# kris927b/TextBlaster

Hardware: AMD Instinct MI355X
Metric: documents/sec through full C4+Gopher+langID pipeline at 1/2/4/8 MI355X (higher is better)
Workload: dtype bf16

## Files before the change

csrc/common/docproc.h:

```cpp
#pragma once
#include <type_traits>

#include "devplan.h"
#include "hash.h"
#include "langid.h"
#include "par.h"
#include "uax29.h"
#include "ucd.h"

namespace tb {

enum : int {
  PH_START = 0, PH_DECODE, PH_DICT, PH_PREFIX_HASH, PH_WORDS, PH_LINES, PH_GQ, PH_GR_LINES, PH_GR_WORDS,
  PH_GR_TOP, PH_GR_DUP, PH_FW, PH_LID, PH_GR_DUP_WALK, PH_GR_DUP_CANON, PH_GR_TOP_CANON,
  PH_C4_LOREM = 16, PH_C4_DECODE, PH_C4_LINES, PH_C4_CITE, PH_C4_WORDS, PH_C4_CODES, PH_C4_JOIN, PH_C4_SENT,
  PH_GR_NL = 24, PH_GR_LINE_DUP, PH_GR_WH, PH_GR_WCANON, PH_GQ_WORDS, PH_GQ_BYTES, PH_RUST_LINES,
  kPhaseSlots = 32
};

enum : uint32_t {
  DOC_OK = 0,
  DOC_NEEDS_CPU = 1,
  DOC_OVERFLOW = 2,
};
// ... 729 lines not shown
  bool collided = false;
  x.par.for_n(n, [&](uint32_t i) {
    uint32_t c = (uint32_t)(tab[canon[i]] & 0xFFFFFFFFull) - 1u;
    if (c != i && !eq(i, c)) { collided = true; c = i; }
    canon[i] = c;
    res(i, c);
  });
  if (collided) x.set_flag(DOC_NEEDS_CPU);
  x.par.sync();
  x.reset(mark);
}

template <class P, class KeyF, class EqF, class CT>
TB_HD void canonicalize(DocCtx<P>& x, uint32_t n, KeyF&& key, EqF&& eq, CT* canon) {
  canonicalize_res(x, n, key, eq, canon, NoResolve{});
}

template <class P>
TB_HD bool bytes_eq(const uint8_t* b, uint32_t a0, uint32_t a1, uint32_t b0, uint32_t b1) {
  if (a1 - a0 != b1 - b0) return false;
  const uint32_t n = a1 - a0;
  uint32_t i = 0;
  for (; i + 16 <= n; i += 16) {
    uint32_t diff = 0;
#pragma unroll
    for (uint32_t k = 0; k < 16; ++k) diff |= (uint32_t)(b[a0 + i + k] ^ b[b0 + i + k]);
    if (diff) return false;
  }
  uint32_t diff = 0;
  for (; i < n; ++i) diff |= (uint32_t)(b[a0 + i] ^ b[b0 + i]);
  return diff == 0;
}

template <class P, class SpanF>
TB_HD void dup_spans(DocCtx<P>& x, const uint8_t* b, const PHView& ph, uint32_t n, SpanF&& span,
                     int64_t* out_elems, int64_t* out_bytes) {
  if (n <= 1) {
    *out_elems = 0;
    *out_bytes = 0;
    return;
  }
  const auto mark = x.mark();
  uint32_t* canon = x.template alloc_hot<uint32_t>(n + 1);
  if (x.overflow) return;
  canonicalize(
      x, n,
      [&](uint32_t i) {
        uint32_t s, e;
        span(i, s, e);
        return dev_key(span_hash8(x, ph, s, e), e - s);
      },
      [&](uint32_t i, uint32_t j) {
        uint32_t s0, e0, s1, e1;
        span(i, s0, e0);
        span(j, s1, e1);
        return bytes_eq<P>(b, s0, e0, s1, e1);
      },
      canon);
  *out_elems = x.par.template sum<int64_t>(n, [&](uint32_t i) { return canon[i] != i ? (int64_t)1 : (int64_t)0; });
  *out_bytes = x.par.template sum<int64_t>(n, [&](uint32_t i) {
    if (canon[i] == i) return (int64_t)0;
    uint32_t s, e;
    span(i, s, e);
    return (int64_t)(e - s);
  });
  x.reset(mark);
}

template <class F>
TB_HD void lower_bytes(const UcdView& ucd, const Cps& cv, uint32_t s, uint32_t e, F&& push) {
  uint8_t buf[4];
  const PropArr prop = cv.props();
  for (uint32_t k = s; k < e; ++k) {
    uint32_t c = cv.cp(k);
    uint32_t lc;
    if (c == 0x3A3) {
      bool before = false, after = false;
      for (uint32_t j = k; j > s; --j) {
        uint32_t p = prop[j - 1];
        if (p & P16_CASE_IGN) continue;
        before = (p & P_CASED) != 0;
        break;
      }
// ... 310 lines not shown
  uint32_t* segf = x.template alloc_hot<uint32_t>(kChunk + 1);
  if (x.overflow) return 0;
  const PropArr prop = c.props() + s;
  CpsAcc acc{prop};
  uint32_t cnt = 0;
  bool seen = false;
  for (uint32_t base = 0; base < m && cnt < limit; base += kChunk) {
    const uint32_t len = m - base < kChunk ? m - base : kChunk;
    const uint32_t NS = x.par.template compact<int>(
        len, [&](uint32_t i, int&) { const uint32_t g = base + i; return g == 0 || sb_break(acc, (int)m, (int)g); },
        [&](uint32_t i, uint32_t k, int&) { starts[k] = i; });
    x.par.sync();
    const uint32_t first = NS ? starts[0] : len;
    const bool lead_any = x.par.template sum<uint32_t>(first, [&](uint32_t i) {
      return is_ws(prop[base + i]) ? 0u : 1u;
    }) != 0;
    const uint32_t segs = x.par.template sum<uint32_t>(NS, [&](uint32_t k) {
      const uint32_t a = starts[k], bnd = k + 1 < NS ? starts[k + 1] : len;
      uint32_t f = 0;
      for (uint32_t j = a; j < bnd; ++j) if (!is_ws(prop[base + j])) { f = 1; break; }
      segf[k] = f;
      return f;
    });
    x.par.sync();
    if (!seen && lead_any) ++cnt;
    cnt += segs;
    seen = NS ? segf[NS - 1] != 0 : (seen || lead_any);
    x.par.sync();
  }
  x.reset(mark);
  return cnt;
}

template <class P>
TB_HD void gopher_rep_record(DocCtx<P>& x, const DevStep& ds, const uint8_t* b, const Cps& c,
                             const PHView& ph, const Words& w, int64_t* r, bool release_props = false,
                             GrExport* ex = nullptr, const PreDoc* pre = nullptr,
                             const uint8_t* b_export = nullptr, Lines lines = Lines{}) {
  const uint32_t C = c.n;
  const PropArr prop = c.props();
  const OffArr off = c.offs();
  const int width = ds.width;
  uint32_t tcs, tce;
  trim_span(x, prop, C, tcs, tce);
  if (tcs >= tce) {
    x.par.single([&]() {
      for (int k = 0; k < width; ++k) r[k] = 0;
      r[0] = -1;
    });
    return;
  }
  const auto mark = x.mark();
  const uint32_t span = tce - tcs;
  uint32_t* rs;
  uint32_t* rl;
  uint32_t NR;
  if (pre) {
    const uint32_t a = pre->nl_a, e = pre->nl_e;
    rs = pre->nl_pos + a;
    rl = pre->nl_len + a;
    NR = e - a;
  } else if (lines.n > 0) {
    const uint32_t* ls = lines.ls;
    const uint32_t NL = lines.n;
    rs = P::kWaves == 1 ? x.template alloc_hot<uint32_t>(NL + 1) : x.template alloc<uint32_t>(NL + 1);
    rl = P::kWaves == 1 ? x.template alloc_hot<uint32_t>(NL + 1) : x.template alloc<uint32_t>(NL + 1);
    if (x.overflow) return;
// ... 47 lines not shown
  const uint32_t NPR = x.par.template compact<int>(
      NR, [&](uint32_t k, int&) { return rl[k] >= 2; }, [&](uint32_t k, uint32_t q, int&) { prs[q] = k; });
  x.par.sync();
  if (!split_lines)
    dup_spans(x, b, ph, NPR + 1,
              [&](uint32_t q, uint32_t& s0, uint32_t& e0) {
                gr_para_span(rs, rl, prs, off, tcs, tce, NPR, q, s0, e0);
              },
              &para_dup, &para_dup_b);
  if (ex) {
    x.par.single([&]() {
      ex->rs = rs; ex->rl = rl; ex->prs = prs; ex->off = off; ex->ph = ph;
      ex->NR = NR; ex->NPR = NPR; ex->tcs = tcs; ex->tce = tce;
      ex->lines_valid = split_lines ? 1u : 0u;
    });
  }
  x.stamp(PH_GR_LINES);
  x.par.single([&]() {
    r[0] = span;
    r[1] = NPR + 1;
    r[2] = para_dup;
    r[3] = para_dup_b;
    r[4] = NR + 1;
    r[5] = line_dup;
    r[6] = line_dup_b;
  });
  const uint32_t W = w.n;
  const bool ngrams = ds.n_top + ds.n_dup > 0;
  if constexpr (P::kWaves == 1) {
    if (ngrams && W >= kWave16) {
      x.set_flag(DOC_NEEDS_CPU);
      return;
    }
    if (ngrams && ex) {
      const uint64_t base = (x.used + 255) & ~255ull;
      x.par.single([&]() {
        for (int t = 0; t < ds.n_top + ds.n_dup; ++t) r[rec_gr_fixed() + t] = 0;
        ex->bs = w.bs; ex->be = w.be;
        ex->b = b_export ? b_export : b;
        ex->free_base = x.scr + base;
        ex->free_cap = x.cap > base ? x.cap - base : 0;
        ex->W = W;
        ex->valid = x.overflow ? 0u : 1u;
      });
      x.par.sync();
      x.stamp(PH_GR_WORDS);
      x.reset(mark);
      return;
    }
  }
  uint32_t* wid = nullptr;
  uint32_t* WL = nullptr;
  uint64_t* K = nullptr;
  uint64_t* PB = nullptr;
  if (ngrams && pre && pre->wready) {
    wid = pre->wid;
    WL = pre->wl;
    K = pre->wk;
    PB = pre->wpb;
  } else if (ngrams) {
    const uint64_t tab_bytes = 6ull * W + 64;
    wid = ex ? x.template alloc<uint32_t>(W + 1) : x.template alloc_hot_keep<uint32_t>(W + 1, tab_bytes);
    WL = ex ? x.template alloc<uint32_t>(W + 1) : x.template alloc_hot_keep<uint32_t>(W + 1, tab_bytes);
    K = ex ? x.template alloc<uint64_t>(W + 1) : x.template alloc_hot_keep<uint64_t>(W + 1, tab_bytes);
    PB = ex ? x.template alloc<uint64_t>(W + 1) : x.template alloc_hot_keep<uint64_t>(W + 1, tab_bytes);
    const auto mw = x.mark();
    uint64_t* wh = x.template alloc_hot_hi<uint64_t>(W + 1);
    if (x.overflow) return;
    x.par.for_n(W, [&](uint32_t k) { wh[k] = span_hash8(x, ph, w.bs[k], w.be[k]); });
    x.par.sync();
    x.stamp(PH_GR_WH);
    canonicalize(
        x, W, [&](uint32_t k) { return dev_key(wh[k], w.be[k] - w.bs[k]); },
        [&](uint32_t i, uint32_t j) { return bytes_eq<P>(b, w.bs[i], w.be[i], w.bs[j], w.be[j]); }, wid);
    x.stamp(PH_GR_WCANON);
    const uint32_t totl = x.par.template scan<uint32_t>(
        W, 0u, [](uint32_t a, uint32_t c2) { return a + c2; },
        [&](uint32_t k) { return w.be[k] - w.bs[k]; }, [&](uint32_t k, uint32_t e) { WL[k] = e; });
    x.par.single([&]() { WL[W] = totl; });
    x.par.sync();
    x.par.for_n(W + 1, [&](uint32_t k) { PB[k] = x.powb(WL[k]); });
    const uint64_t ktot = x.par.template scan<uint64_t>(
        W, 0ull, [](uint64_t a, uint64_t c2) { return a + c2; },
        [&](uint32_t j) { return wh[j] * x.ipowb(WL[j + 1]); }, [&](uint32_t k, uint64_t e) { K[k] = e; });
    x.par.single([&]() { K[W] = ktot; });
    x.par.sync();
    x.reset(mw);
    if (x.overflow) return;
  }
  x.stamp(PH_GR_WORDS);
  if (release_props) x.release_hi();
  if (ngrams) {
    const DupGrams dg{wid, WL, K, PB, w.bs, w.be, b};
    if (ds.n_top > 0 && ex) {
      x.par.single([&]() { for (int t = 0; t < ds.n_top; ++t) r[rec_gr_fixed() + t] = 0; });
    } else if (ds.n_top > 0) {
      int max_top = 0;
      for (int t = 0; t < ds.n_top; ++t) max_top = ds.top_n[t] > max_top ? ds.top_n[t] : max_top;
      const auto m2 = x.mark();
      uint32_t* ga = x.template alloc_hot_keep<uint32_t>(W + 1, 6ull * W + 64);
      uint32_t* gb = x.template alloc_hot_keep<uint32_t>(W + 1, 6ull * W + 64);
      if (x.overflow) return;
      x.par.single([&]() { for (int t = 0; t < ds.n_top; ++t) r[rec_gr_fixed() + t] = 0; });
      const uint32_t* gprev = wid;
      for (uint32_t n = 1; n <= (uint32_t)max_top && W >= n; ++n) {
        const uint32_t G = W - n + 1;
        const uint32_t* gc = wid;
        uint32_t* cnt = (n == 1 || !(n & 1)) ? ga : gb;
        if (n > 1) {
          uint32_t* gcur = (n & 1) ? ga : gb;
          canonicalize(
              x, G, [&](uint32_t p) { return mix64(((uint64_t)gprev[p] << 32) ^ (uint64_t)wid[p + n - 1] ^ ((uint64_t)n << 60)); },
              [&](uint32_t p, uint32_t q) { return gprev[p] == gprev[q] && wid[p + n - 1] == wid[q + n - 1]; }, gcur);
          gc = gcur;
          gprev = gcur;
          x.stamp(PH_GR_TOP_CANON);
        }
        bool wanted = false;
        for (int t = 0; t < ds.n_top; ++t) wanted |= ds.top_n[t] == (int32_t)n;
        if (!wanted) continue;
        x.par.for_n(G, [&](uint32_t p) { cnt[p] = 0; });
        x.par.sync();
        x.par.for_n(G, [&](uint32_t p) { P::add32(&cnt[gc[p]], 1u); });
        x.par.sync();
        const uint32_t maxc = x.par.template max<uint32_t>(G, 0u, [&](uint32_t p) { return cnt[p]; });
        int64_t v = 0;
        if (maxc > 1) {
          const uint32_t maxlen = x.par.template max<uint32_t>(G, 0u, [&](uint32_t p) {
            return cnt[p] == maxc ? (WL[p + n] - WL[p] + n - 1) : 0u;
          });
          v = (int64_t)maxlen * (int64_t)maxc;
        }
        x.par.single([&]() {
          for (int t = 0; t < ds.n_top; ++t) if (ds.top_n[t] == (int32_t)n) r[rec_gr_fixed() + t] = v;
        });
        x.par.sync();
      }
      x.reset(m2);
    }
    x.stamp(PH_GR_TOP);
    if (ex) {
      const uint64_t base = (x.used + 255) & ~255ull;
      x.par.single([&]() {
        for (int t = 0; t < ds.n_dup; ++t) r[rec_gr_fixed() + ds.n_top + t] = 0;
        ex->wid = wid; ex->WL = WL; ex->K = K; ex->PB = PB; ex->bs = w.bs; ex->be = w.be;
        ex->b = b_export ? b_export : b;
        ex->free_base = x.scr + base;
        ex->free_cap = x.cap > base ? x.cap - base : 0;
        ex->W = W;
        ex->valid = x.overflow ? 0u : 1u;
      });
      x.par.sync();
    } else if (ds.n_dup > 0) {
      const uint32_t SW = (W + 31) / 32 + 1;
      const int nd = ds.n_dup;
      auto gsize = [&](int t) -> uint32_t {
        const uint32_t n = (uint32_t)ds.dup_n[t];
        return (n == 0 || W < n) ? 0u : W - n + 1;
      };
      uint32_t gtot = 0;
      for (int t = 0; t < nd; ++t) gtot += gsize(t);
      const auto m3 = x.mark();
      uint32_t* bits = x.template alloc_hot<uint32_t>(2 * (uint64_t)SW * (uint64_t)nd);
      using GcT = std::conditional_t<P::kWaves == 1, uint16_t, uint32_t>;
      GcT* gcall = x.template alloc_hot_keep<GcT>((uint64_t)gtot + 1, 6ull * W + 64);
      if (x.overflow) return;
      x.par.for_n(2 * SW * (uint32_t)nd, [&](uint32_t i) { bits[i] = 0; });
      x.par.sync();
      uint32_t gb = 0;
      for (int t = 0; t < nd; ++t) {
        const uint32_t n = (uint32_t)ds.dup_n[t];
        const uint32_t G = gsize(t);
        if (G == 0) continue;
        GcT* gc = gcall + gb;
        uint32_t* R = bits + (uint32_t)t * 2 * SW + SW;
        gb += G;
        auto mark_rep = [&](uint32_t p, uint32_t g) {
          if (g != p) {
            P::or32(&R[p >> 5], 1u << (p & 31));
            P::or32(&R[g >> 5], 1u << (g & 31));
          }
        };
        if constexpr (P::kWaves != 1) {
          canonicalize_res(
              x, G, [&](uint32_t p) { return dg.key(p, n); }, [&](uint32_t p, uint32_t q) { return dg.eq(p, q, n); },
              gc, mark_rep);
          x.stamp(PH_GR_DUP_CANON);
        } else {
          canonicalize(
              x, G, [&](uint32_t p) { return dg.key(p, n); }, [&](uint32_t p, uint32_t q) { return dg.eq(p, q, n); },
              gc);
          x.stamp(PH_GR_DUP_CANON);
          x.par.for_n(G, [&](uint32_t p) { mark_rep(p, gc[p]); });
          x.par.sync();
        }
      }
      auto walk = [&](uint32_t t, bool wave) -> int64_t {
        const uint32_t G = gsize((int)t);
        if (G == 0) return 0;
        uint32_t base = 0;
        for (uint32_t u = 0; u < t; ++u) base += gsize((int)u);
        uint32_t* sn = bits + t * 2 * SW;
        const uint32_t n = (uint32_t)ds.dup_n[t];
        return wave ? dup_walk_wave(x.par, G, n, gcall + base, sn + SW, sn, WL)
                    : dup_walk(G, n, gcall + base, sn + SW, sn, WL);
      };
      if constexpr (P::kWaves > 1) {
        for (uint32_t t = x.par.wave_index(); t < (uint32_t)nd; t += P::kWaves) {
          const int64_t rep = walk(t, true);
          if (x.par.lane == 0) r[rec_gr_fixed() + ds.n_top + t] = rep;
        }
      } else {
        x.par.for_n((uint32_t)nd, [&](uint32_t t) { r[rec_gr_fixed() + ds.n_top + t] = walk(t, false); });
      }
      x.par.sync();
      x.stamp(PH_GR_DUP_WALK);
      x.reset(m3);
      x.stamp(PH_GR_DUP);
    }
  }
  x.reset(mark);
}

template <class P, class KeyF>
TB_HD uint32_t repeat_candidates(DocCtx<P>& x, uint32_t n, KeyF&& key, uint32_t* bm, uint32_t bw, uint32_t* list) {
  const uint32_t mask = bw * 32u - 1u;
  uint32_t* once = bm;
  uint32_t* twice = bm + bw;
  x.par.for_n(2 * bw, [&](uint32_t i) { bm[i] = 0; });
  x.par.sync();
  x.par.for_n(n, [&](uint32_t i) {
    const uint32_t h = (uint32_t)(key(i) >> 20) & mask;
    const uint32_t bit = 1u << (h & 31u);
    if (P::fetch_or32(&once[h >> 5], bit) & bit) P::or32(&twice[h >> 5], bit);
  });
  x.par.sync();
  const uint32_t nc = x.par.template compact<int>(
      n,
      [&](uint32_t i, int&) {
        const uint32_t h = (uint32_t)(key(i) >> 20) & mask;
        return ((twice[h >> 5] >> (h & 31u)) & 1u) != 0;
      },
      [&](uint32_t i, uint32_t k, int&) { list[k] = i; });
  x.par.sync();
  return nc;
}

TB_HD uint32_t cand_bitmap_words(uint32_t n) {
  uint32_t w = 32;
  while (w * 4u < n) w <<= 1;
  return w;
// ... 1032 lines not shown
    x.par.single([&]() { *wout = wk; });
  }
  x.stamp(PH_C4_CODES);
  uint32_t* joff = x.template alloc_hot<uint32_t>(NLn + 1);
  if (x.overflow) { x.set_flag(DOC_NEEDS_CPU | DOC_OVERFLOW); return; }
  uint32_t Jtot = x.par.template scan<uint32_t>(
      NLn, 0u, [](uint32_t a, uint32_t b2) { return a + b2; },
      [&](uint32_t k) { return code[k] == 0 ? plen[k] + 1 : 0u; }, [&](uint32_t k, uint32_t e) { joff[k] = e; });
  if (Jtot > 0) Jtot -= 1;
  uint8_t* Jb = x.template alloc_global<uint8_t>(Jtot + 1);
  if (x.overflow) { x.set_flag(DOC_NEEDS_CPU | DOC_OVERFLOW); return; }
  x.par.sync();
  x.par.for_n(C, [&](uint32_t j) {
    const uint32_t nb = kept_bytes(j);
    if (!nb || code[lid[j]] != 0) return;
    const uint32_t k = lid[j];
    uint8_t* d = Jb + joff[k] + (Pw[j] - Pw[la[k]]);
    for (uint32_t q = 0; q < nb; ++q) d[q] = b[off[j] + q];
  });
  x.par.for_n(NLn, [&](uint32_t k) {
    if (code[k] == 0 && joff[k] + plen[k] < Jtot) Jb[joff[k] + plen[k]] = '\n';
  });
  x.par.sync();
  x.stamp(PH_C4_JOIN);
  c4_finish(x, c4, n, Jb, Jtot, s_long, s_punct, s_few, r, src);
}


#ifndef TB_HOT_PROPS
#define TB_HOT_PROPS 1
#endif
constexpr bool kHotProps = TB_HOT_PROPS != 0;

template <class P, bool kWithLid = true, bool kPre = false>
TB_HD void analyze_stage(DocCtx<P>& x, const DevStage& st, const DevPlan& plan,
                         const LidTables& lid, const uint8_t* b, uint32_t n, StageOut& out) {
  bool need_words = false, need_lines = false, need_ph = false, need_lid = false;
  for (int s = 0; s < st.n_steps; ++s) {
    const int k = st.steps[s].kind;
    if (k == DK_GOPHER_QUALITY) need_words = need_lines = true;
    if (k == DK_GOPHER_REP) need_words = need_ph = true;
    if (k == DK_FINEWEB) need_words = need_lines = need_ph = true;
    if (k == DK_LANGID) need_lid = true;
  }
  x.stamp(PH_START);
  if (out.line_stats) x.par.single([&]() { out.line_stats[0] = kLineStatsNone; });
  uint32_t ndict = 0;
  Cps c;
  if constexpr (kPre) {
    c.n = out.pre->C;
    c.off = out.pre->off;
    c.prop = out.pre->prop;
    c.b = b;
    c.nb = n;
    ndict = out.pre->dict;
  } else {
    c = decode(x, b, n, kHotProps, &ndict);
  }
  if (x.overflow) { x.set_flag(DOC_NEEDS_CPU | DOC_OVERFLOW); return; }
  x.stamp(PH_DECODE);
  const uint32_t C = c.n;
  const uint32_t* dict_marks = nullptr;
  uint32_t wfix = kNoWords;
  if (ndict && need_words) {
    bool fw_only = true;
    for (int s = 0; s < st.n_steps; ++s)
      fw_only &= st.steps[s].kind != DK_GOPHER_QUALITY && st.steps[s].kind != DK_GOPHER_REP;
    if (!kPre) dict_marks = out.dict.marks(out.doc);
    if (!kPre && !dict_marks && fw_only) wfix = out.dict.nwords(out.doc);
    if (!dict_marks && wfix == kNoWords) {
      if constexpr (kWithLid) {
        for (int s = 0; s < st.n_steps; ++s) {
          const DevStep& ds = st.steps[s];
          if (ds.kind == DK_LANGID && lid.E)
            langid_record(x, b, n, lid, out.rec + (int64_t)ds.rec_prefix * out.ndocs + (int64_t)out.doc * ds.width);
        }
      }
      x.set_flag(DOC_NEEDS_CPU);
      return;
    }
  }
  x.stamp(PH_DICT);
  PHView ph;
  if (need_ph) ph = prefix_hash8(x, b, n);
  x.stamp(PH_PREFIX_HASH);
  Words w;
  if (need_words) {
    w = words(x, c, kPre ? out.pre : nullptr, dict_marks);
  }
  x.stamp(PH_WORDS);
  Lines L;
  if (need_lines) L = rust_lines(x, c);
  if (x.overflow) { x.set_flag(DOC_NEEDS_CPU | DOC_OVERFLOW); return; }
  x.stamp(PH_RUST_LINES);
  if (out.line_stats && need_words && need_lines) export_line_stats(x, c, w, L, n, out.line_stats);
  x.stamp(PH_LINES);
  const uint32_t W = w.n;
  const PropArr prop = c.props();
  const OffArr off = c.offs();

  int n_gr = 0;
  for (int s = 0; s < st.n_steps; ++s) n_gr += st.steps[s].kind == DK_GOPHER_REP;
  int gr_seen = 0;
  for (int so = 0; so < 2 * st.n_steps; ++so) {
    const int s = so % st.n_steps;
    const DevStep& ds = st.steps[s];
    if ((so < st.n_steps) == (ds.kind == DK_GOPHER_REP)) continue;
    int64_t* r = out.rec + (int64_t)ds.rec_prefix * out.ndocs + (int64_t)out.doc * ds.width;
    if (ds.kind == DK_GOPHER_QUALITY) {
      const DevStopSet& ss = plan.stops[ds.stop_set];
      const UcdView ucd = x.ucd;
      auto lo32 = [](uint64_t v) { return (int64_t)(v & 0xFFFFFFFFull); };
      auto hi32 = [](uint64_t v) { return (int64_t)(v >> 32); };
      int64_t sum_chars = 0;
      const uint64_t as = x.par.template sum<uint64_t>(W, [&](uint32_t k) {
        const uint32_t a = w.cs[k], e = w.ce[k];
        return ((uint64_t)(e - a) << 32) | ((uint64_t)w.alpha[k] << 16) |
// ... 18 lines not shown
        if (c0 == 0xE2) return (uint64_t)(i + 2 < n && b[i + 1] == 0x80 && b[i + 2] == 0xA6);
        if (c0 != '.' || (i > 0 && b[i - 1] == '.')) return (uint64_t)0;
        uint32_t j = i;
        while (j < n && b[j] == '.') ++j;
        return (uint64_t)((j - i) / 3);
      });
      x.stamp(PH_GQ_BYTES);
      const int64_t nhash = hi32(he), nell = lo32(he);
      const uint64_t be = x.par.template sum<uint64_t>(L.n, [&](uint32_t k) {
        const uint32_t ls = L.ls[k], le = L.le[k];
        uint32_t j = ls;
        while (j < le && is_ws(prop[j])) ++j;
        const uint32_t l0 = j < le ? c.lead(j) : 0u;
        const uint64_t bul = (l0 == '-' || (l0 == 0xE2 && c.cp(j) == 0x2022)) ? 1 : 0;
        j = le;
        while (j > ls && is_ws(prop[j - 1])) --j;
        const uint32_t E = off[j], S = off[ls];
        uint64_t ell = 0;
        if (E - S >= 3) {
          const bool dots = b[E - 3] == '.' && b[E - 2] == '.' && b[E - 1] == '.';
          const bool uell = b[E - 3] == 0xE2 && b[E - 2] == 0x80 && b[E - 1] == 0xA6;
          ell = (dots || uell) ? 1 : 0;
        }
        return (bul << 32) | ell;
      });
      const int64_t bullet = hi32(be), ell_lines = lo32(be);
      x.par.single([&]() {
        r[0] = W; r[1] = sum_chars; r[2] = nhash; r[3] = nell; r[4] = L.n;
        r[5] = bullet; r[6] = ell_lines; r[7] = alpha; r[8] = stop;
      });
      x.stamp(PH_GQ);
    } else if (ds.kind == DK_GOPHER_REP) {
      ++gr_seen;
      gopher_rep_record(x, ds, b, c, ph, w, r, kHotProps && gr_seen == n_gr, n_gr == 1 ? out.gr_export : nullptr,
                        kPre ? out.pre : nullptr, out.b_global, L);
    } else if (ds.kind == DK_FINEWEB) {
      const auto mark = x.mark();
      uint32_t* nb = x.template alloc<uint32_t>(L.n + 1);
      if (x.overflow) { x.set_flag(DOC_NEEDS_CPU | DOC_OVERFLOW); return; }
      const uint32_t NB = x.par.template compact<int>(
          L.n,
          [&](uint32_t k, int&) {
            for (uint32_t j = L.ls[k]; j < L.le[k]; ++j) if (!is_ws(prop[j])) return true;
            return false;
          },
          [&](uint32_t k, uint32_t q, int&) { nb[q] = k; });
      x.par.sync();
      int64_t stop_end = x.par.template sum<int64_t>(NB, [&](uint32_t q) {
        uint32_t k = nb[q];
        uint32_t j = L.le[k];
        while (j > L.ls[k] && is_ws(prop[j - 1])) --j;
        uint32_t last = c.cp(j - 1);
        for (int t = 0; t < ds.n_stop_chars; ++t) if (ds.stop_chars[t] == last) return (int64_t)1;
        return (int64_t)0;
      });
      int64_t shrt = x.par.template sum<int64_t>(NB, [&](uint32_t q) {
        uint32_t k = nb[q];
        return (int64_t)((int64_t)(L.le[k] - L.ls[k]) <= ds.short_line_length);
      });
      int64_t dup_e = 0, dup_b = 0;
      dup_spans(x, b, ph, NB,
                [&](uint32_t q, uint32_t& s0, uint32_t& e0) { s0 = off[L.ls[nb[q]]]; e0 = off[L.le[nb[q]]]; },
                &dup_e, &dup_b);
      int64_t nl = x.par.template sum<int64_t>(C, [&](uint32_t i) { return (int64_t)c.is_lf(i); });
      x.par.single([&]() {
        r[0] = NB; r[1] = stop_end; r[2] = shrt; r[3] = dup_b; r[4] = (int64_t)C - nl; r[5] = nl; r[6] = W;
      });
      x.reset(mark);
// ... 22 lines not shown
```

csrc/hip/stage.hip:

```cpp
#include <algorithm>

#include "kernel_common.h"

namespace {

#define TB_STAGE_KERNEL(NAME, ATTR)                                                                   \
  __global__ __launch_bounds__(64) ATTR void NAME(                                                   \
      const DevPlan* __restrict__ plan, const DevStage* __restrict__ stage, const uint8_t* __restrict__ bytes, \
      const int64_t* __restrict__ off, const int32_t* __restrict__ perm, int32_t ndocs, char* scratch,        \
      const int64_t* __restrict__ scratch_off, const uint64_t* __restrict__ pw, uint32_t pw_n, DevTables tabs, \
      int64_t* rec, uint32_t* flags, uint32_t lds_bytes, uint64_t* prof,                               \
      const uint8_t* __restrict__ dead, uint32_t* line_stats, GrExport* gr_export, DictIn dict) {      \
    const int doc = perm ? perm[blockIdx.x] : (int)blockIdx.x;                                        \
    if (doc >= ndocs || (dead && dead[doc])) return;                                                  \
    DocCtx<WavePar> x = make_ctx(tabs, pw, pw_n, scratch, scratch_off, doc, (int)blockIdx.x, flags, lds_bytes, prof);   \
    const uint32_t n = (uint32_t)(off[doc + 1] - off[doc]);                                           \
    lds_ascii_props(x);                                                                               \
    const uint8_t* b = lds_text(x, bytes + off[doc], n);                                              \
    StageOut out{rec, (uint32_t)ndocs, (uint32_t)doc};                                                \
    if (line_stats) out.line_stats = line_stats + line_stats_base(off[doc], doc);                     \
    if (gr_export) { out.gr_export = gr_export + blockIdx.x; out.b_global = bytes + off[doc]; }       \
    out.dict = dict;                                                                                  \
    analyze_stage<WavePar, false>(x, *stage, *plan, LidTables{}, b, n, out);  \
  }

#ifndef TB_STAGE_WPE
#define TB_STAGE_WPE 8
#endif
TB_STAGE_KERNEL(k_stage_analyze_wave, __attribute__((amdgpu_waves_per_eu(TB_STAGE_WPE, 8))))

#ifndef TB_BLK_WPE
#define TB_BLK_WPE 6
#endif
#if TB_BLK_WPE > 0
#define TB_BLK_ATTR __attribute__((amdgpu_waves_per_eu(TB_BLK_WPE, 8)))
#else
#define TB_BLK_ATTR
#endif

template <int NT, bool kPre = false>
__device__ __forceinline__ void stage_blk_body(
    const DevPlan* __restrict__ plan, const DevStage* __restrict__ stage, const uint8_t* __restrict__ bytes,
    const int64_t* __restrict__ off, const int32_t* __restrict__ perm, int32_t ndocs, char* scratch,
    const int64_t* __restrict__ scratch_off, const uint64_t* __restrict__ pw, uint32_t pw_n, DevTables tabs,
    int64_t* rec, uint32_t* flags, uint32_t lds_bytes, uint64_t* prof, const uint8_t* __restrict__ dead,
    GrExport* gr_export, int32_t n_split, uint32_t split_bytes, uint32_t* line_stats, const PreDoc* pre,
    int32_t n_pre, DictIn dict) {
  const int doc = perm[blockIdx.x];
  if (doc >= ndocs || (dead && dead[doc])) return;
  DocCtx<BlockPar<NT>> x =
      make_ctx<BlockPar<NT>>(tabs, pw, pw_n, scratch, scratch_off, doc, (int)blockIdx.x, flags, lds_bytes, prof);
  x.par.xs = g_block_xs;
  lds_ascii_props(x);
  const uint8_t* b = bytes + off[doc];
  const uint32_t n = (uint32_t)(off[doc + 1] - off[doc]);
  StageOut out{rec, (uint32_t)ndocs, (uint32_t)doc};
  out.dict = dict;
  if (line_stats) out.line_stats = line_stats + line_stats_base(off[doc], doc);
  if constexpr (kPre) {
    if (pre[blockIdx.x].n != n) return;
    out.pre = pre + blockIdx.x;
  }
// ... 7 lines not shown
      const int64_t* __restrict__ off, const int32_t* __restrict__ perm, int32_t ndocs, char* scratch,         \
      const int64_t* __restrict__ scratch_off, const uint64_t* __restrict__ pw, uint32_t pw_n, DevTables tabs,  \
      int64_t* rec, uint32_t* flags, uint32_t lds_bytes, uint64_t* prof, const uint8_t* __restrict__ dead,   \
      GrExport* gr_export, int32_t n_split, uint32_t split_bytes, uint32_t* line_stats,                \
      const PreDoc* pre, int32_t n_pre, DictIn dict) {                                                 \
    stage_blk_body<NT, PRE>(plan, stage, bytes, off, perm, ndocs, scratch, scratch_off, pw, pw_n, tabs, rec, flags, \
                       lds_bytes, prof, dead, gr_export, n_split, split_bytes, line_stats, pre, n_pre, dict); \
  }
TB_STAGE_BLK_KERNEL(k_stage_analyze_blk, kBlockThreads, false)
TB_STAGE_BLK_KERNEL(k_stage_analyze_blk_pre, kBlockThreads, true)

}

extern "C" {

int tb_abi_version() { return 27; }
size_t tb_sizeof_tables() { return sizeof(TbTables); }
size_t tb_sizeof_docs() { return sizeof(TbDocs); }
size_t tb_sizeof_work() { return sizeof(TbWork); }
size_t tb_sizeof_dict_in() { return sizeof(DictIn); }
size_t tb_sizeof_dict_lines() { return sizeof(DictLines); }
size_t tb_sizeof_plan() { return sizeof(DevPlan); }
size_t tb_sizeof_stage() { return sizeof(DevStage); }
int tb_block_threads() { return kBlockThreads; }
int tb_phase_slots() { return kPhaseSlots; }
int tb_stage_waves() { return TB_STAGE_WPE; }

int tb_stage_analyze(hipStream_t stream, const void* plan, const void* stage, const TbDocs* d, const TbWork* w,
                     const TbTables* tb, uint32_t* line_stats, void* gr_export, const DictIn* dict) {
  const uint32_t lds_bytes = w->lds_bytes;
  if (d->ndocs <= 0) return 0;
  const int32_t nblocks = d->n_launch <= 0 ? d->ndocs : d->n_launch;
  if (lds_bytes > kMaxLdsPerDoc) return (int)hipErrorInvalidValue;
  auto kern = k_stage_analyze_wave;
  if (lds_bytes > 65536)
    (void)hipFuncSetAttribute((const void*)kern, hipFuncAttributeMaxDynamicSharedMemorySize, (int)lds_bytes);
  hipLaunchKernelGGL(kern, dim3(nblocks), dim3(64), lds_bytes, stream, (const DevPlan*)plan,
                     (const DevStage*)stage, d->bytes, d->off, d->perm, d->ndocs, w->scratch, w->scratch_off, tb->pw,
                     tb->pw_n, tb->ucd, w->rec, w->flags, lds_bytes, w->prof, d->dead, line_stats, (GrExport*)gr_export,
                     dict ? *dict : DictIn{});
  return (int)hipGetLastError();
}

int tb_stage_analyze_blk(hipStream_t stream, const void* plan, const void* stage, const TbDocs* d, const TbWork* w,
                         const TbTables* tb, void* gr_export, int32_t n_split, uint32_t split_bytes,
                         uint32_t* line_stats, const void* pre, const DictIn* dict) {
  const int32_t nblocks = d->n_launch;
  const uint32_t lds_bytes = w->lds_bytes;
  if (nblocks <= 0) return 0;
  if (!d->perm || lds_bytes > kMaxLdsPerBlk || n_split < 0 || n_split > nblocks) return (int)hipErrorInvalidValue;
  auto kern = pre ? k_stage_analyze_blk_pre : k_stage_analyze_blk;
  if (lds_bytes > 65536)
    (void)hipFuncSetAttribute((const void*)kern, hipFuncAttributeMaxDynamicSharedMemorySize, (int)lds_bytes);
  hipLaunchKernelGGL(kern, dim3(nblocks), dim3(kBlockThreads), lds_bytes, stream, (const DevPlan*)plan,
                     (const DevStage*)stage, d->bytes, d->off, d->perm, d->ndocs, w->scratch, w->scratch_off, tb->pw,
                     tb->pw_n, tb->ucd, w->rec, w->flags, lds_bytes, w->prof, d->dead, (GrExport*)gr_export, n_split,
                     split_bytes, line_stats, (const PreDoc*)pre, pre ? nblocks : 0, dict ? *dict : DictIn{});
  return (int)hipGetLastError();
}

}

namespace {

__global__ __launch_bounds__(kBlockThreads) TB_BLK_ATTR void k_gr_dup_split(
    const DevStage* __restrict__ stage, int32_t gr_step, const int32_t* __restrict__ perm, int32_t n_split,
    int32_t n_tasks, int32_t ndocs, const GrExport* __restrict__ ex, const uint64_t* __restrict__ pw, uint32_t pw_n,
// ... 70 lines not shown
```

Before: 13.76 million.

## Add wave-level duplicate span check and export-specialized stage kernel skipping prefix hash

For single-wave documents with at most 64 spans, duplicate line/paragraph detection now runs through a register and ballot lane comparison instead of hash-based canonicalize with scratch allocation. The wave path also keys canonicalize on the first and last bytes of each span rather than the prefix hash. A new kernel variant, specialized at compile time for the gopher export path, skips prefix_hash8 and compiles out the in-kernel n-gram code, which reduces both computation and register pressure. The risks are quadratic work on the lane path when many spans collide, and more key collisions from the ends-based key, which fall back to full byte comparison.

```diff
diff --git a/csrc/common/docproc.h b/csrc/common/docproc.h
--- a/csrc/common/docproc.h
+++ b/csrc/common/docproc.h
@@ -785,6 +785,54 @@
   return diff == 0;
 }
 
+TB_HD uint64_t span_ends_key(const uint8_t* b, uint32_t s, uint32_t e) {
+  const uint32_t len = e - s, m = len < 8u ? len : 8u;
+  uint64_t head = 0, tail = 0;
+  for (uint32_t k = 0; k < m; ++k) {
+    head |= (uint64_t)b[s + k] << (8u * k);
+    tail |= (uint64_t)b[e - m + k] << (8u * k);
+  }
+  return dev_key(head ^ (tail * kHashBase), len);
+}
+
+#if defined(__HIPCC__)
+template <class P, class SpanF>
+__device__ __forceinline__ void dup_spans_lanes(DocCtx<P>& x, const uint8_t* b, uint32_t n, SpanF&& span,
+                                                int64_t* out_elems, int64_t* out_bytes) {
+  const uint32_t lane = x.par.lane;
+  uint32_t s = 0, len = 0, lo = 0, hi = 0;
+  if (lane < n) {
+    uint32_t e;
+    span(lane, s, e);
+    len = e - s;
+    const uint32_t m = len < 8u ? len : 8u;
+#pragma unroll
+    for (uint32_t k = 0; k < 4; ++k) {
+      if (k < m) lo |= (uint32_t)b[s + k] << (8u * k);
+      if (k + 4 < m) hi |= (uint32_t)b[s + k + 4] << (8u * k);
+    }
+  }
+  uint64_t dup = 0;
+  for (uint32_t i = 0; i + 1 < n; ++i) {
+    if ((dup >> i) & 1ull) continue;
+    const uint32_t si = (uint32_t)__builtin_amdgcn_readlane((int)s, (int)i);
+    const uint32_t li = (uint32_t)__builtin_amdgcn_readlane((int)len, (int)i);
+    const uint32_t loi = (uint32_t)__builtin_amdgcn_readlane((int)lo, (int)i);
+    const uint32_t hii = (uint32_t)__builtin_amdgcn_readlane((int)hi, (int)i);
+    bool hit = lane > i && lane < n && !((dup >> lane) & 1ull) && len == li && lo == loi && hi == hii;
+    if (hit) {
+      uint32_t diff = 0;
+#pragma unroll 1
+      for (uint32_t k = 8; k < li; ++k) diff |= (uint32_t)(b[si + k] ^ b[s + k]);
+      hit = diff == 0;
+    }
+    dup |= __ballot(hit);
+  }
+  *out_elems = (int64_t)__popcll(dup);
+  *out_bytes = (int64_t)x.par.template wave_sum<uint32_t>(((dup >> lane) & 1ull) ? len : 0u);
+}
+#endif
+
 template <class P, class SpanF>
 TB_HD void dup_spans(DocCtx<P>& x, const uint8_t* b, const PHView& ph, uint32_t n, SpanF&& span,
                      int64_t* out_elems, int64_t* out_bytes) {
@@ -793,6 +841,14 @@
     *out_bytes = 0;
     return;
   }
+#if defined(__HIPCC__)
+  if constexpr (P::kWaves == 1) {
+    if (n <= 64) {
+      dup_spans_lanes(x, b, n, span, out_elems, out_bytes);
+      return;
+    }
+  }
+#endif
   const auto mark = x.mark();
   uint32_t* canon = x.template alloc_hot<uint32_t>(n + 1);
   if (x.overflow) return;
@@ -801,7 +857,8 @@
       [&](uint32_t i) {
         uint32_t s, e;
         span(i, s, e);
-        return dev_key(span_hash8(x, ph, s, e), e - s);
+        if constexpr (P::kWaves == 1) return span_ends_key(b, s, e);
+        else return dev_key(span_hash8(x, ph, s, e), e - s);
       },
       [&](uint32_t i, uint32_t j) {
         uint32_t s0, e0, s1, e1;
@@ -1178,7 +1235,7 @@
   return cnt;
 }
 
-template <class P>
+template <class P, bool kExport = false>
 TB_HD void gopher_rep_record(DocCtx<P>& x, const DevStep& ds, const uint8_t* b, const Cps& c,
                              const PHView& ph, const Words& w, int64_t* r, bool release_props = false,
                              GrExport* ex = nullptr, const PreDoc* pre = nullptr,
@@ -1292,7 +1349,13 @@
       x.set_flag(DOC_NEEDS_CPU);
       return;
     }
-    if (ngrams && ex) {
+    if constexpr (kExport) {
+      if (!(ngrams && ex)) {
+        x.set_flag(DOC_NEEDS_CPU);
+        return;
+      }
+    }
+    if (kExport || (ngrams && ex)) {
       const uint64_t base = (x.used + 255) & ~255ull;
       x.par.single([&]() {
         for (int t = 0; t < ds.n_top + ds.n_dup; ++t) r[rec_gr_fixed() + t] = 0;
@@ -1309,174 +1372,176 @@
       return;
     }
   }
-  uint32_t* wid = nullptr;
-  uint32_t* WL = nullptr;
-  uint64_t* K = nullptr;
-  uint64_t* PB = nullptr;
-  if (ngrams && pre && pre->wready) {
-    wid = pre->wid;
-    WL = pre->wl;
-    K = pre->wk;
-    PB = pre->wpb;
-  } else if (ngrams) {
-    const uint64_t tab_bytes = 6ull * W + 64;
-    wid = ex ? x.template alloc<uint32_t>(W + 1) : x.template alloc_hot_keep<uint32_t>(W + 1, tab_bytes);
-    WL = ex ? x.template alloc<uint32_t>(W + 1) : x.template alloc_hot_keep<uint32_t>(W + 1, tab_bytes);
-    K = ex ? x.template alloc<uint64_t>(W + 1) : x.template alloc_hot_keep<uint64_t>(W + 1, tab_bytes);
-    PB = ex ? x.template alloc<uint64_t>(W + 1) : x.template alloc_hot_keep<uint64_t>(W + 1, tab_bytes);
-    const auto mw = x.mark();
-    uint64_t* wh = x.template alloc_hot_hi<uint64_t>(W + 1);
-    if (x.overflow) return;
-    x.par.for_n(W, [&](uint32_t k) { wh[k] = span_hash8(x, ph, w.bs[k], w.be[k]); });
-    x.par.sync();
-    x.stamp(PH_GR_WH);
-    canonicalize(
-        x, W, [&](uint32_t k) { return dev_key(wh[k], w.be[k] - w.bs[k]); },
-        [&](uint32_t i, uint32_t j) { return bytes_eq<P>(b, w.bs[i], w.be[i], w.bs[j], w.be[j]); }, wid);
-    x.stamp(PH_GR_WCANON);
-    const uint32_t totl = x.par.template scan<uint32_t>(
-        W, 0u, [](uint32_t a, uint32_t c2) { return a + c2; },
-        [&](uint32_t k) { return w.be[k] - w.bs[k]; }, [&](uint32_t k, uint32_t e) { WL[k] = e; });
-    x.par.single([&]() { WL[W] = totl; });
-    x.par.sync();
-    x.par.for_n(W + 1, [&](uint32_t k) { PB[k] = x.powb(WL[k]); });
-    const uint64_t ktot = x.par.template scan<uint64_t>(
-        W, 0ull, [](uint64_t a, uint64_t c2) { return a + c2; },
-        [&](uint32_t j) { return wh[j] * x.ipowb(WL[j + 1]); }, [&](uint32_t k, uint64_t e) { K[k] = e; });
-    x.par.single([&]() { K[W] = ktot; });
-    x.par.sync();
-    x.reset(mw);
-    if (x.overflow) return;
-  }
-  x.stamp(PH_GR_WORDS);
-  if (release_props) x.release_hi();
-  if (ngrams) {
-    const DupGrams dg{wid, WL, K, PB, w.bs, w.be, b};
-    if (ds.n_top > 0 && ex) {
-      x.par.single([&]() { for (int t = 0; t < ds.n_top; ++t) r[rec_gr_fixed() + t] = 0; });
-    } else if (ds.n_top > 0) {
-      int max_top = 0;
-      for (int t = 0; t < ds.n_top; ++t) max_top = ds.top_n[t] > max_top ? ds.top_n[t] : max_top;
-      const auto m2 = x.mark();
-      uint32_t* ga = x.template alloc_hot_keep<uint32_t>(W + 1, 6ull * W + 64);
-      uint32_t* gb = x.template alloc_hot_keep<uint32_t>(W + 1, 6ull * W + 64);
+  if constexpr (!kExport) {
+    uint32_t* wid = nullptr;
+    uint32_t* WL = nullptr;
+    uint64_t* K = nullptr;
+    uint64_t* PB = nullptr;
+    if (ngrams && pre && pre->wready) {
+      wid = pre->wid;
+      WL = pre->wl;
+      K = pre->wk;
+      PB = pre->wpb;
+    } else if (ngrams) {
+      const uint64_t tab_bytes = 6ull * W + 64;
+      wid = ex ? x.template alloc<uint32_t>(W + 1) : x.template alloc_hot_keep<uint32_t>(W + 1, tab_bytes);
+      WL = ex ? x.template alloc<uint32_t>(W + 1) : x.template alloc_hot_keep<uint32_t>(W + 1, tab_bytes);
+      K = ex ? x.template alloc<uint64_t>(W + 1) : x.template alloc_hot_keep<uint64_t>(W + 1, tab_bytes);
+      PB = ex ? x.template alloc<uint64_t>(W + 1) : x.template alloc_hot_keep<uint64_t>(W + 1, tab_bytes);
+      const auto mw = x.mark();
+      uint64_t* wh = x.template alloc_hot_hi<uint64_t>(W + 1);
       if (x.overflow) return;
-      x.par.single([&]() { for (int t = 0; t < ds.n_top; ++t) r[rec_gr_fixed() + t] = 0; });
-      const uint32_t* gprev = wid;
-      for (uint32_t n = 1; n <= (uint32_t)max_top && W >= n; ++n) {
-        const uint32_t G = W - n + 1;
-        const uint32_t* gc = wid;
-        uint32_t* cnt = (n == 1 || !(n & 1)) ? ga : gb;
-        if (n > 1) {
-          uint32_t* gcur = (n & 1) ? ga : gb;
-          canonicalize(
-              x, G, [&](uint32_t p) { return mix64(((uint64_t)gprev[p] << 32) ^ (uint64_t)wid[p + n - 1] ^ ((uint64_t)n << 60)); },
-              [&](uint32_t p, uint32_t q) { return gprev[p] == gprev[q] && wid[p + n - 1] == wid[q + n - 1]; }, gcur);
-          gc = gcur;
-          gprev = gcur;
-          x.stamp(PH_GR_TOP_CANON);
+      x.par.for_n(W, [&](uint32_t k) { wh[k] = span_hash8(x, ph, w.bs[k], w.be[k]); });
+      x.par.sync();
+      x.stamp(PH_GR_WH);
+      canonicalize(
+          x, W, [&](uint32_t k) { return dev_key(wh[k], w.be[k] - w.bs[k]); },
+          [&](uint32_t i, uint32_t j) { return bytes_eq<P>(b, w.bs[i], w.be[i], w.bs[j], w.be[j]); }, wid);
+      x.stamp(PH_GR_WCANON);
+      const uint32_t totl = x.par.template scan<uint32_t>(
+          W, 0u, [](uint32_t a, uint32_t c2) { return a + c2; },
+          [&](uint32_t k) { return w.be[k] - w.bs[k]; }, [&](uint32_t k, uint32_t e) { WL[k] = e; });
+      x.par.single([&]() { WL[W] = totl; });
+      x.par.sync();
+      x.par.for_n(W + 1, [&](uint32_t k) { PB[k] = x.powb(WL[k]); });
+      const uint64_t ktot = x.par.template scan<uint64_t>(
+          W, 0ull, [](uint64_t a, uint64_t c2) { return a + c2; },
+          [&](uint32_t j) { return wh[j] * x.ipowb(WL[j + 1]); }, [&](uint32_t k, uint64_t e) { K[k] = e; });
+      x.par.single([&]() { K[W] = ktot; });
+      x.par.sync();
+      x.reset(mw);
+      if (x.overflow) return;
+    }
+    x.stamp(PH_GR_WORDS);
+    if (release_props) x.release_hi();
+    if (ngrams) {
+      const DupGrams dg{wid, WL, K, PB, w.bs, w.be, b};
+      if (ds.n_top > 0 && ex) {
+        x.par.single([&]() { for (int t = 0; t < ds.n_top; ++t) r[rec_gr_fixed() + t] = 0; });
+      } else if (ds.n_top > 0) {
+        int max_top = 0;
+        for (int t = 0; t < ds.n_top; ++t) max_top = ds.top_n[t] > max_top ? ds.top_n[t] : max_top;
+        const auto m2 = x.mark();
+        uint32_t* ga = x.template alloc_hot_keep<uint32_t>(W + 1, 6ull * W + 64);
+        uint32_t* gb = x.template alloc_hot_keep<uint32_t>(W + 1, 6ull * W + 64);
+        if (x.overflow) return;
+        x.par.single([&]() { for (int t = 0; t < ds.n_top; ++t) r[rec_gr_fixed() + t] = 0; });
+        const uint32_t* gprev = wid;
+        for (uint32_t n = 1; n <= (uint32_t)max_top && W >= n; ++n) {
+          const uint32_t G = W - n + 1;
+          const uint32_t* gc = wid;
+          uint32_t* cnt = (n == 1 || !(n & 1)) ? ga : gb;
+          if (n > 1) {
+            uint32_t* gcur = (n & 1) ? ga : gb;
+            canonicalize(
+                x, G, [&](uint32_t p) { return mix64(((uint64_t)gprev[p] << 32) ^ (uint64_t)wid[p + n - 1] ^ ((uint64_t)n << 60)); },
+                [&](uint32_t p, uint32_t q) { return gprev[p] == gprev[q] && wid[p + n - 1] == wid[q + n - 1]; }, gcur);
+            gc = gcur;
+            gprev = gcur;
+            x.stamp(PH_GR_TOP_CANON);
+          }
+          bool wanted = false;
+          for (int t = 0; t < ds.n_top; ++t) wanted |= ds.top_n[t] == (int32_t)n;
+          if (!wanted) continue;
+          x.par.for_n(G, [&](uint32_t p) { cnt[p] = 0; });
+          x.par.sync();
+          x.par.for_n(G, [&](uint32_t p) { P::add32(&cnt[gc[p]], 1u); });
+          x.par.sync();
+          const uint32_t maxc = x.par.template max<uint32_t>(G, 0u, [&](uint32_t p) { return cnt[p]; });
+          int64_t v = 0;
+          if (maxc > 1) {
+            const uint32_t maxlen = x.par.template max<uint32_t>(G, 0u, [&](uint32_t p) {
+              return cnt[p] == maxc ? (WL[p + n] - WL[p] + n - 1) : 0u;
+            });
+            v = (int64_t)maxlen * (int64_t)maxc;
+          }
+          x.par.single([&]() {
+            for (int t = 0; t < ds.n_top; ++t) if (ds.top_n[t] == (int32_t)n) r[rec_gr_fixed() + t] = v;
+          });
+          x.par.sync();
         }
-        bool wanted = false;
-        for (int t = 0; t < ds.n_top; ++t) wanted |= ds.top_n[t] == (int32_t)n;
-        if (!wanted) continue;
-        x.par.for_n(G, [&](uint32_t p) { cnt[p] = 0; });
-        x.par.sync();
-        x.par.for_n(G, [&](uint32_t p) { P::add32(&cnt[gc[p]], 1u); });
-        x.par.sync();
-        const uint32_t maxc = x.par.template max<uint32_t>(G, 0u, [&](uint32_t p) { return cnt[p]; });
-        int64_t v = 0;
-        if (maxc > 1) {
-          const uint32_t maxlen = x.par.template max<uint32_t>(G, 0u, [&](uint32_t p) {
-            return cnt[p] == maxc ? (WL[p + n] - WL[p] + n - 1) : 0u;
-          });
-          v = (int64_t)maxlen * (int64_t)maxc;
-        }
+        x.reset(m2);
+      }
+      x.stamp(PH_GR_TOP);
+      if (ex) {
+        const uint64_t base = (x.used + 255) & ~255ull;
         x.par.single([&]() {
-          for (int t = 0; t < ds.n_top; ++t) if (ds.top_n[t] == (int32_t)n) r[rec_gr_fixed() + t] = v;
+          for (int t = 0; t < ds.n_dup; ++t) r[rec_gr_fixed() + ds.n_top + t] = 0;
+          ex->wid = wid; ex->WL = WL; ex->K = K; ex->PB = PB; ex->bs = w.bs; ex->be = w.be;
+          ex->b = b_export ? b_export : b;
+          ex->free_base = x.scr + base;
+          ex->free_cap = x.cap > base ? x.cap - base : 0;
+          ex->W = W;
+          ex->valid = x.overflow ? 0u : 1u;
         });
         x.par.sync();
-      }
-      x.reset(m2);
-    }
-    x.stamp(PH_GR_TOP);
-    if (ex) {
-      const uint64_t base = (x.used + 255) & ~255ull;
-      x.par.single([&]() {
-        for (int t = 0; t < ds.n_dup; ++t) r[rec_gr_fixed() + ds.n_top + t] = 0;
-        ex->wid = wid; ex->WL = WL; ex->K = K; ex->PB = PB; ex->bs = w.bs; ex->be = w.be;
-        ex->b = b_export ? b_export : b;
-        ex->free_base = x.scr + base;
-        ex->free_cap = x.cap > base ? x.cap - base : 0;
-        ex->W = W;
-        ex->valid = x.overflow ? 0u : 1u;
-      });
-      x.par.sync();
-    } else if (ds.n_dup > 0) {
-      const uint32_t SW = (W + 31) / 32 + 1;
-      const int nd = ds.n_dup;
-      auto gsize = [&](int t) -> uint32_t {
-        const uint32_t n = (uint32_t)ds.dup_n[t];
-        return (n == 0 || W < n) ? 0u : W - n + 1;
-      };
-      uint32_t gtot = 0;
-      for (int t = 0; t < nd; ++t) gtot += gsize(t);
-      const auto m3 = x.mark();
-      uint32_t* bits = x.template alloc_hot<uint32_t>(2 * (uint64_t)SW * (uint64_t)nd);
-      using GcT = std::conditional_t<P::kWaves == 1, uint16_t, uint32_t>;
-      GcT* gcall = x.template alloc_hot_keep<GcT>((uint64_t)gtot + 1, 6ull * W + 64);
-      if (x.overflow) return;
-      x.par.for_n(2 * SW * (uint32_t)nd, [&](uint32_t i) { bits[i] = 0; });
-      x.par.sync();
-      uint32_t gb = 0;
-      for (int t = 0; t < nd; ++t) {
-        const uint32_t n = (uint32_t)ds.dup_n[t];
-        const uint32_t G = gsize(t);
-        if (G == 0) continue;
-        GcT* gc = gcall + gb;
-        uint32_t* R = bits + (uint32_t)t * 2 * SW + SW;
-        gb += G;
-        auto mark_rep = [&](uint32_t p, uint32_t g) {
-          if (g != p) {
-            P::or32(&R[p >> 5], 1u << (p & 31));
-            P::or32(&R[g >> 5], 1u << (g & 31));
+      } else if (ds.n_dup > 0) {
+        const uint32_t SW = (W + 31) / 32 + 1;
+        const int nd = ds.n_dup;
+        auto gsize = [&](int t) -> uint32_t {
+          const uint32_t n = (uint32_t)ds.dup_n[t];
+          return (n == 0 || W < n) ? 0u : W - n + 1;
+        };
+        uint32_t gtot = 0;
+        for (int t = 0; t < nd; ++t) gtot += gsize(t);
+        const auto m3 = x.mark();
+        uint32_t* bits = x.template alloc_hot<uint32_t>(2 * (uint64_t)SW * (uint64_t)nd);
+        using GcT = std::conditional_t<P::kWaves == 1, uint16_t, uint32_t>;
+        GcT* gcall = x.template alloc_hot_keep<GcT>((uint64_t)gtot + 1, 6ull * W + 64);
+        if (x.overflow) return;
+        x.par.for_n(2 * SW * (uint32_t)nd, [&](uint32_t i) { bits[i] = 0; });
+        x.par.sync();
+        uint32_t gb = 0;
+        for (int t = 0; t < nd; ++t) {
+          const uint32_t n = (uint32_t)ds.dup_n[t];
+          const uint32_t G = gsize(t);
+          if (G == 0) continue;
+          GcT* gc = gcall + gb;
+          uint32_t* R = bits + (uint32_t)t * 2 * SW + SW;
+          gb += G;
+          auto mark_rep = [&](uint32_t p, uint32_t g) {
+            if (g != p) {
+              P::or32(&R[p >> 5], 1u << (p & 31));
+              P::or32(&R[g >> 5], 1u << (g & 31));
+            }
+          };
+          if constexpr (P::kWaves != 1) {
+            canonicalize_res(
+                x, G, [&](uint32_t p) { return dg.key(p, n); }, [&](uint32_t p, uint32_t q) { return dg.eq(p, q, n); },
+                gc, mark_rep);
+            x.stamp(PH_GR_DUP_CANON);
+          } else {
+            canonicalize(
+                x, G, [&](uint32_t p) { return dg.key(p, n); }, [&](uint32_t p, uint32_t q) { return dg.eq(p, q, n); },
+                gc);
+            x.stamp(PH_GR_DUP_CANON);
+            x.par.for_n(G, [&](uint32_t p) { mark_rep(p, gc[p]); });
+            x.par.sync();
           }
+        }
+        auto walk = [&](uint32_t t, bool wave) -> int64_t {
+          const uint32_t G = gsize((int)t);
+          if (G == 0) return 0;
+          uint32_t base = 0;
+          for (uint32_t u = 0; u < t; ++u) base += gsize((int)u);
+          uint32_t* sn = bits + t * 2 * SW;
+          const uint32_t n = (uint32_t)ds.dup_n[t];
+          return wave ? dup_walk_wave(x.par, G, n, gcall + base, sn + SW, sn, WL)
+                      : dup_walk(G, n, gcall + base, sn + SW, sn, WL);
         };
-        if constexpr (P::kWaves != 1) {
-          canonicalize_res(
-              x, G, [&](uint32_t p) { return dg.key(p, n); }, [&](uint32_t p, uint32_t q) { return dg.eq(p, q, n); },
-              gc, mark_rep);
-          x.stamp(PH_GR_DUP_CANON);
+        if constexpr (P::kWaves > 1) {
+          for (uint32_t t = x.par.wave_index(); t < (uint32_t)nd; t += P::kWaves) {
+            const int64_t rep = walk(t, true);
+            if (x.par.lane == 0) r[rec_gr_fixed() + ds.n_top + t] = rep;
+          }
         } else {
-          canonicalize(
-              x, G, [&](uint32_t p) { return dg.key(p, n); }, [&](uint32_t p, uint32_t q) { return dg.eq(p, q, n); },
-              gc);
-          x.stamp(PH_GR_DUP_CANON);
-          x.par.for_n(G, [&](uint32_t p) { mark_rep(p, gc[p]); });
-          x.par.sync();
+          x.par.for_n((uint32_t)nd, [&](uint32_t t) { r[rec_gr_fixed() + ds.n_top + t] = walk(t, false); });
         }
-      }
-      auto walk = [&](uint32_t t, bool wave) -> int64_t {
-        const uint32_t G = gsize((int)t);
-        if (G == 0) return 0;
-        uint32_t base = 0;
-        for (uint32_t u = 0; u < t; ++u) base += gsize((int)u);
-        uint32_t* sn = bits + t * 2 * SW;
-        const uint32_t n = (uint32_t)ds.dup_n[t];
-        return wave ? dup_walk_wave(x.par, G, n, gcall + base, sn + SW, sn, WL)
-                    : dup_walk(G, n, gcall + base, sn + SW, sn, WL);
-      };
-      if constexpr (P::kWaves > 1) {
-        for (uint32_t t = x.par.wave_index(); t < (uint32_t)nd; t += P::kWaves) {
-          const int64_t rep = walk(t, true);
-          if (x.par.lane == 0) r[rec_gr_fixed() + ds.n_top + t] = rep;
-        }
-      } else {
-        x.par.for_n((uint32_t)nd, [&](uint32_t t) { r[rec_gr_fixed() + ds.n_top + t] = walk(t, false); });
-      }
-      x.par.sync();
-      x.stamp(PH_GR_DUP_WALK);
-      x.reset(m3);
-      x.stamp(PH_GR_DUP);
+        x.par.sync();
+        x.stamp(PH_GR_DUP_WALK);
+        x.reset(m3);
+        x.stamp(PH_GR_DUP);
+      }
     }
   }
   x.reset(mark);
@@ -2575,7 +2640,7 @@
 #endif
 constexpr bool kHotProps = TB_HOT_PROPS != 0;
 
-template <class P, bool kWithLid = true, bool kPre = false>
+template <class P, bool kWithLid = true, bool kPre = false, bool kExport = false>
 TB_HD void analyze_stage(DocCtx<P>& x, const DevStage& st, const DevPlan& plan,
                          const LidTables& lid, const uint8_t* b, uint32_t n, StageOut& out) {
   bool need_words = false, need_lines = false, need_ph = false, need_lid = false;
@@ -2585,6 +2650,16 @@
     if (k == DK_GOPHER_REP) need_words = need_ph = true;
     if (k == DK_FINEWEB) need_words = need_lines = need_ph = true;
     if (k == DK_LANGID) need_lid = true;
+  }
+  if constexpr (P::kWaves == 1) {
+    int n_gr = 0;
+    bool gr_ngrams = false;
+    for (int s = 0; s < st.n_steps; ++s) {
+      if (st.steps[s].kind != DK_GOPHER_REP) continue;
+      ++n_gr;
+      gr_ngrams |= st.steps[s].n_top + st.steps[s].n_dup > 0;
+    }
+    need_ph = !kExport && gr_ngrams && !(n_gr == 1 && out.gr_export);
   }
   x.stamp(PH_START);
   if (out.line_stats) x.par.single([&]() { out.line_stats[0] = kLineStatsNone; });
@@ -2625,7 +2700,9 @@
   }
   x.stamp(PH_DICT);
   PHView ph;
-  if (need_ph) ph = prefix_hash8(x, b, n);
+  if constexpr (!kExport) {
+    if (need_ph) ph = prefix_hash8(x, b, n);
+  }
   x.stamp(PH_PREFIX_HASH);
   Words w;
   if (need_words) {
@@ -2710,8 +2787,8 @@
       x.stamp(PH_GQ);
     } else if (ds.kind == DK_GOPHER_REP) {
       ++gr_seen;
-      gopher_rep_record(x, ds, b, c, ph, w, r, kHotProps && gr_seen == n_gr, n_gr == 1 ? out.gr_export : nullptr,
-                        kPre ? out.pre : nullptr, out.b_global, L);
+      gopher_rep_record<P, kExport>(x, ds, b, c, ph, w, r, kHotProps && gr_seen == n_gr,
+                                    n_gr == 1 ? out.gr_export : nullptr, kPre ? out.pre : nullptr, out.b_global, L);
     } else if (ds.kind == DK_FINEWEB) {
       const auto mark = x.mark();
       uint32_t* nb = x.template alloc<uint32_t>(L.n + 1);
diff --git a/csrc/hip/stage.hip b/csrc/hip/stage.hip
--- a/csrc/hip/stage.hip
+++ b/csrc/hip/stage.hip
@@ -4,7 +4,7 @@
 
 namespace {
 
-#define TB_STAGE_KERNEL(NAME, ATTR)                                                                   \
+#define TB_STAGE_KERNEL(NAME, ATTR, EXPORT)                                                           \
   __global__ __launch_bounds__(64) ATTR void NAME(                                                   \
       const DevPlan* __restrict__ plan, const DevStage* __restrict__ stage, const uint8_t* __restrict__ bytes, \
       const int64_t* __restrict__ off, const int32_t* __restrict__ perm, int32_t ndocs, char* scratch,        \
@@ -21,13 +21,15 @@
     if (line_stats) out.line_stats = line_stats + line_stats_base(off[doc], doc);                     \
     if (gr_export) { out.gr_export = gr_export + blockIdx.x; out.b_global = bytes + off[doc]; }       \
     out.dict = dict;                                                                                  \
-    analyze_stage<WavePar, false>(x, *stage, *plan, LidTables{}, b, n, out);  \
+                                                                   \
+    analyze_stage<WavePar, false, false, EXPORT>(x, *stage, *plan, LidTables{}, b, n, out);           \
   }
 
 #ifndef TB_STAGE_WPE
 #define TB_STAGE_WPE 8
 #endif
-TB_STAGE_KERNEL(k_stage_analyze_wave, __attribute__((amdgpu_waves_per_eu(TB_STAGE_WPE, 8))))
+TB_STAGE_KERNEL(k_stage_analyze_wave, __attribute__((amdgpu_waves_per_eu(TB_STAGE_WPE, 8))), false)
+TB_STAGE_KERNEL(k_stage_analyze_wave_ex, __attribute__((amdgpu_waves_per_eu(TB_STAGE_WPE, 8))), true)
 
 #ifndef TB_BLK_WPE
 #define TB_BLK_WPE 6
@@ -101,7 +103,7 @@
   if (d->ndocs <= 0) return 0;
   const int32_t nblocks = d->n_launch <= 0 ? d->ndocs : d->n_launch;
   if (lds_bytes > kMaxLdsPerDoc) return (int)hipErrorInvalidValue;
-  auto kern = k_stage_analyze_wave;
+  auto kern = gr_export ? k_stage_analyze_wave_ex : k_stage_analyze_wave;
   if (lds_bytes > 65536)
     (void)hipFuncSetAttribute((const void*)kern, hipFuncAttributeMaxDynamicSharedMemorySize, (int)lds_bytes);
   hipLaunchKernelGGL(kern, dim3(nblocks), dim3(64), lds_bytes, stream, (const DevPlan*)plan,
```

Measured after the change: 14.35 million (median of 6 runs). 4.3% higher.
